# aje220/OptiMOBO

Measured on AMD Instinct MI355X. Metric: EHVI candidate evals/sec at n_train=512, 2-obj; 1/2/4/8-GPU scaling, higher is better.
Workload: dtype f64; 1 GPU; 2-obj EHVI (reference mode), ZDT1 surrogate, n_train=512, n_var=6, 2^20 Sobol candidates per GPU (BASELINE config 3); n_train=512, n_var=6, n_obj=2, candidates_per_gpu=1048576, global_batch=1048576, parallelism=dp1, train_box=x_1 in [0, 1], x_2..x_6 in [0, 0.3]

## Files before the change

### include/optimobo_hip.h

```cpp
#ifndef OPTIMOBO_HIP_H
#define OPTIMOBO_HIP_H

#include <stdint.h>

#ifdef __cplusplus
extern "C" {
#endif

#define OMB_ABI_VERSION 1
#define OMB_MAX_OBJ 8
#define OMB_MAX_DIM 256
#define OMB_MAX_TRAIN 1024
#define OMB_MAX_TRAIN_DENSE 16384
#define OMB_HVI_PATHS_CHUNK 262144
#define OMB_NONDOM_SETS 16
#define OMB_NONDOM_POINTS 16777216

enum {
  OMB_OK = 0,
  OMB_EINVAL = -1,
  OMB_EHIP = -2,
  OMB_ENOMEM = -3,
  OMB_ESTATE = -4,
  OMB_EUNSUP = -5,
// ... 35 lines not shown
  OMB_DEBUG_COV_TABLE = 2,
  OMB_DEBUG_FUSED_CHAIN = 3,
  OMB_DEBUG_ARGMAX_PASSES = 4,
  OMB_DEBUG_CHOL_MODE = 5,
  OMB_DEBUG_TIMING_STRIDE = 6,
  OMB_DEBUG_COV_FUSED = 8,
  OMB_DEBUG_SELECT_SEQ = 9,
  OMB_DEBUG_SYRK_GLDS = 10,
  OMB_DEBUG_BOXES_KD = 11,
  OMB_DEBUG_POSTERIOR_ALL_VAR = 12,
  OMB_DEBUG_POSTERIOR_MEAN_KERNEL = 13,
  OMB_DEBUG_PATHS_LIBCOS = 14,
  OMB_DEBUG_HVI_PATHS_CHUNK = 15,
  OMB_DEBUG_ARGMAX_PRUNE = 16,
  OMB_DEBUG_ARGMAX_SCREEN = 17,
  OMB_DEBUG_ARGMAX_STAGED = 18
};
int omb_debug_set(omb_ctx* ctx, int what, int64_t value);

int omb_set_gp(omb_ctx* ctx, int obj, int kernel, int n, int d, const double* X_dev,
               const double* lengthscale_host, double variance, const double* alpha_dev,
               const double* Linv_dev);

int omb_kernel_block(omb_ctx* ctx, int obj, const double* Xc_dev, int64_t N, double* K_dev);

int omb_posterior(omb_ctx* ctx, int n_obj, const double* Xc_dev, int64_t N, double* mu_dev,
                  double* var_dev);

int omb_posterior_screen(omb_ctx* ctx, const double* Xc_dev, int64_t N, int n_obj, double* mu_out_dev,
                          double* eps_out_dev);

// ... 24 lines not shown
                  int C, const int32_t* box_off_host, const uint16_t* boxes_dev, double* out_dev);
int omb_hvi_paths_grad(omb_ctx* ctx, int k, int S, int d, const double* y_dev, const double* dy_dev, int64_t ld,
                       int64_t N, const double* coords_dev, int C, const int32_t* box_off_host,
                       const uint16_t* boxes_dev, double* out_dev, double* grad_dev, double* t_dev,
                       double* tgrad_dev);
#define OMB_CON_VIOLATION 1u
int omb_hvi_paths_con(omb_ctx* ctx, int k, int S, int n_con, const double* y_dev, int64_t ld, int64_t N,
                      const double* coords_dev, int C, const int32_t* box_off_host, const uint16_t* boxes_dev,
                      double eta, unsigned flags, double* out_dev, double* u_dev);

int omb_nondominated(omb_ctx* ctx, int k, int S, const double* y_dev, int64_t ld, int64_t N, uint8_t* mask_dev,
                     int64_t ldm, int64_t* count_dev);
int omb_nondominated_stats(omb_ctx* ctx, int64_t* survivors_host, int* rounds_host);
int omb_argmax_prune_stats(omb_ctx* ctx, int64_t* stats_host);
int omb_argmax_stage_stats(omb_ctx* ctx, int64_t* stats_host);

int omb_hvpoi(omb_ctx* ctx, const double* mu_dev, const double* var_dev, int64_t ld, int64_t N,
              const double* cells_dev, int C, double* out_dev);

int omb_expdec(omb_ctx* ctx, int k, const double* mu_dev, const double* var_dev, int64_t ld, int64_t N,
               const double* cache_dev, int M, int scal_id, const double* params_host,
               const double* weights_host, const double* ideal_host, const double* max_host,
               double agg_min, double* out_dev);

int omb_ei(omb_ctx* ctx, const double* mu_dev, const double* var_dev, int64_t N, double best,
           double var_eps, double* out_dev);
int omb_ei_ext(omb_ctx* ctx, int kind, int k, const double* mu_dev, const double* var_dev, int64_t ld, int64_t N,
               double best, double var_eps, double pof_eps, double* out_dev);

int omb_feasibility(omb_ctx* ctx, int c, const double* mu_dev, const double* var_dev, int64_t ld, int64_t N,
// ... 97 lines not shown
```

### optimobo_amd/_lib.py

```python
import ctypes
import os

HERE = os.path.dirname(os.path.abspath(__file__))
LIB_PATH = os.environ.get("OMB_LIB_PATH") or os.path.join(HERE, "liboptimobo_hip.so")

OMB_OK, OMB_EINVAL, OMB_EHIP, OMB_ENOMEM, OMB_ESTATE, OMB_EUNSUP, OMB_ENOTPD = 0, -1, -2, -3, -4, -5, -6
ERROR_NAMES = {OMB_EINVAL: "OMB_EINVAL", OMB_EHIP: "OMB_EHIP", OMB_ENOMEM: "OMB_ENOMEM",
               OMB_ESTATE: "OMB_ESTATE", OMB_EUNSUP: "OMB_EUNSUP", OMB_ENOTPD: "OMB_ENOTPD"}
KERNEL_MATERN52, KERNEL_RBF = 0, 1
EHVI_REFERENCE, EHVI_TEXTBOOK, EHVI_SIGMA = 0, 1, 2
EI_PLAIN, EI_PARETO, EI_CONSTRAINED = 0, 1, 2
EA_EI, EA_PARETO_EI = 0, 1
DEBUG_SPIN_LIMIT = 1
DEBUG_COV_TABLE = 2
DEBUG_FUSED_CHAIN = 3
DEBUG_ARGMAX_PASSES = 4
DEBUG_CHOL_MODE = 5
DEBUG_TIMING_STRIDE = 6
DEBUG_COV_FUSED = 8
DEBUG_SELECT_SEQ = 9
DEBUG_SYRK_GLDS = 10
DEBUG_BOXES_KD = 11
DEBUG_POSTERIOR_ALL_VAR = 12
DEBUG_POSTERIOR_MEAN_KERNEL = 13
DEBUG_PATHS_LIBCOS = 14
DEBUG_HVI_PATHS_CHUNK = 15
DEBUG_ARGMAX_PRUNE = 16
DEBUG_ARGMAX_SCREEN = 17
DEBUG_ARGMAX_STAGED = 18
MAX_OBJ, MAX_DIM, MAX_TRAIN, MAX_TRAIN_DENSE = 8, 256, 1024, 16384
CON_VIOLATION = 1
HVI_PATHS_CHUNK = 1 << 18
NONDOM_SETS = 16
NONDOM_POINTS = 1 << 24

_p = ctypes.c_void_p
_d = ctypes.c_double
_i = ctypes.c_int
_i64 = ctypes.c_int64
_dp = ctypes.POINTER(ctypes.c_double)

SIGNATURES = {
    "omb_abi_version": (_i, []),
    "omb_create": (_i, [_i, ctypes.POINTER(_p)]),
# ... 9 lines not shown
    "omb_posterior_screen": (_i, [_p, _p, _i64, _i, _p, _p]),
    "omb_posterior_screen_list": (_i, [_p, _p, _i64, _p, _p, _i, _p, _p]),
    "omb_ehvi2d": (_i, [_p, _p, _p, _i64, _i64, _p, _i, _dp, _d, _d, _i, _p]),
    "omb_ehvi3d_mc": (_i, [_p, _p, _p, _i64, _i64, _p, _i, _dp, _d, _p, _p]),
    "omb_ehvi_mc": (_i, [_p, _i, _p, _p, _i64, _i64, _p, _i, _dp, _d, _p, _p]),
    "omb_ehvi_boxes": (_i, [_p, _i, _p, _p, _i64, _i64, _p, _i, _p, _i, _p]),
    "omb_ehvi_boxes_k": (_i, [_p, _i, _p, _p, _i64, _i64, _p, _i, _p, _i, _p]),
    "omb_hvi_boxes": (_i, [_p, _i, _p, _i64, _i64, _p, _i, _p, _i, _p]),
    "omb_hvi_paths": (_i, [_p, _i, _i, _p, _i64, _i64, _p, _i, _p, _p, _p]),
    "omb_hvi_paths_grad": (_i, [_p, _i, _i, _i, _p, _p, _i64, _i64, _p, _i, _p, _p, _p, _p, _p, _p]),
    "omb_hvi_paths_con": (_i, [_p, _i, _i, _i, _p, _i64, _i64, _p, _i, _p, _p, _d, ctypes.c_uint, _p, _p]),
    "omb_nondominated": (_i, [_p, _i, _i, _p, _i64, _i64, _p, _i64, _p]),
    "omb_nondominated_stats": (_i, [_p, ctypes.POINTER(_i64), ctypes.POINTER(_i)]),
    "omb_argmax_prune_stats": (_i, [_p, ctypes.POINTER(_i64)]),
    "omb_argmax_stage_stats": (_i, [_p, ctypes.POINTER(_i64)]),
    "omb_hvpoi": (_i, [_p, _p, _p, _i64, _i64, _p, _i, _p]),
    "omb_expdec": (_i, [_p, _i, _p, _p, _i64, _i64, _p, _i, _i, _dp, _dp, _dp, _dp, _d, _p]),
    "omb_ei": (_i, [_p, _p, _p, _i64, _d, _d, _p]),
    "omb_ei_ext": (_i, [_p, _i, _i, _p, _p, _i64, _i64, _d, _d, _d, _p]),
    "omb_feasibility": (_i, [_p, _i, _p, _p, _i64, _i64, _d, _p, _p]),
    "omb_log_ei": (_i, [_p, _i, _i, _p, _p, _i64, _i64, _d, _d, _d, _p]),
    "omb_log_ehvi_boxes": (_i, [_p, _i, _p, _p, _i64, _i64, _p, _i, _p, _i, _p]),
    "omb_log_feasibility": (_i, [_p, _i, _p, _p, _i64, _i64, _d, _p, _p]),
    "omb_mes": (_i, [_p, _i, _p, _p, _i64, _i64, _p, _i, _p]),
    "omb_argmax_dev": (_i, [_p, _p, _i64, _i64, _p]),
    "omb_argmax": (_i, [_p, _p, _i64, _i64, _dp, ctypes.POINTER(_i64)]),
    "omb_plan_ehvi2d": (_i, [_p, _p, _i, _dp, _d, _d, _i]),
    "omb_plan_ehvi3d_mc": (_i, [_p, _p, _i, _dp, _d]),
    "omb_plan_ehvi_mc": (_i, [_p, _i, _p, _i, _dp, _d]),
    "omb_plan_ehvi_boxes": (_i, [_p, _i, _p, _i, _p, _i]),
# ... 72 lines not shown
```

### optimobo_amd/csrc/omb_acquisition.hip

```cpp
#include <math.h>

#include "omb_internal.h"
#include "omb_math.h"

namespace omb {

constexpr int kAcqThreads = 256;

static unsigned acq_grid(int64_t N) {
  int64_t b = (N + kAcqThreads - 1) / kAcqThreads;
  if (b > 65536) b = 65536;
  return (unsigned)(b < 1 ? 1 : b);
}

int ehvi2d_lanes(int64_t N) { return N >= (1 << 19) ? 1 : (N >= (1 << 16) ? 2 : 4); }

template <int L>
__global__ __launch_bounds__(kAcqThreads) void ehvi2d_kernel(const double* __restrict__ mu,
                                                             const double* __restrict__ var, int64_t ld, int64_t N,
                                                             const double* __restrict__ pf, int P, double r0,
                                                             double r1, double s00, double s01, int mode,
                                                             double* __restrict__ out) {
  extern __shared__ double sm[];
  double* y1 = sm;
// ... 657 lines not shown
    off += (bytes + 15) / 16 * 16;
    return base ? base + o : nullptr;
  };
  ws->partials = reinterpret_cast<double*>(take(sizeof(double) * 2 * 2 * kArgmaxMaxBlocks));
  ws->tau = reinterpret_cast<double*>(take(sizeof(double) * 2));
  ws->counts = reinterpret_cast<int32_t*>(take(sizeof(int32_t) * 4));
  ws->seed_idx = reinterpret_cast<int32_t*>(take(sizeof(int32_t) * ((N + kPruneStride - 1) / kPruneStride)));
  ws->surv_idx = reinterpret_cast<int32_t*>(take(sizeof(int32_t) * N));
  ws->block_cnt = reinterpret_cast<int32_t*>(take(sizeof(int32_t) * ((N + kPruneBlock - 1) / kPruneBlock)));
  ws->keep = reinterpret_cast<uint8_t*>(take(N));
  ws->ubm = reinterpret_cast<double*>(take(sizeof(double) * N));
  ws->scr_mu = reinterpret_cast<double*>(take(sizeof(double) * 2 * N));
  ws->scr_eps = reinterpret_cast<double*>(take(sizeof(double) * 2 * N));
  ws->list_a = reinterpret_cast<int32_t*>(take(sizeof(int32_t) * N));
  ws->block_cnt_b = reinterpret_cast<int32_t*>(take(sizeof(int32_t) * ((N + kPruneBlock - 1) / kPruneBlock)));
  ws->stats_host = nullptr;
  return off;
}

int64_t prune_ws_bytes(int64_t N) {
  PruneWs ws;
  return prune_ws_layout(nullptr, N, &ws);
}

void prune_ws_carve(void* base, int64_t N, PruneWs* ws) { prune_ws_layout(static_cast<char*>(base), N, ws); }

__global__ __launch_bounds__(256) void prune_seed_kernel(int64_t ns, int32_t* __restrict__ seed_idx,
                                                         int32_t* __restrict__ counts) {
  for (int64_t j = (int64_t)blockIdx.x * blockDim.x + threadIdx.x; j < ns; j += (int64_t)gridDim.x * blockDim.x)
    seed_idx[j] = (int32_t)(j * kPruneStride);
// ... 346 lines not shown
      ubm[c] = v;
      const double score = -mc;
      if (score == score && argmax_better(score, c, bv, bi)) {
        bv = score;
        bi = c;
      }
    }
  }
  argmax_wave_block(bv, bi, red_v, red_i);
  if (threadIdx.x == 0) {
    seed_idx[blockIdx.x] = (int32_t)(bi < 0 ? first : bi);
    if (blockIdx.x == 0) counts[0] = (int32_t)gridDim.x;
  }
}

__global__ __launch_bounds__(kPruneBlock) void prune_bound_list_kernel(
    const double* __restrict__ mu0, const double* __restrict__ mu1, const double* __restrict__ eps0,
    const double* __restrict__ eps1, const int32_t* __restrict__ idx_a, const int32_t* __restrict__ count_a,
    int64_t cap, const double* __restrict__ pf, int P, double r0, double sA, double sB,
    const double* __restrict__ tau, uint8_t* __restrict__ keep, int32_t* __restrict__ block_cnt) {
#pragma clang fp contract(off)
  extern __shared__ double sm[];
  double* y1 = sm;
  double* y2 = sm + P + 1;
  __shared__ int wave_cnt[kPruneBlock / 64];
  const int64_t na = min((int64_t)*count_a, cap);
  if ((int64_t)blockIdx.x * kPruneBlock >= na) {
    if (threadIdx.x == 0) block_cnt[blockIdx.x] = 0;
    return;
  }
// ... 41 lines not shown
  for (int w = 0; w < wave; ++w) pos += wave_cnt[w];
  if (k) idx_b[pos] = idx_a[j];
}

hipError_t launch_prune_bound1_seed(hipStream_t stream, const double* mu1, const double* eps1, int64_t N,
                                    const double* pf, int P, double r0, double s00, double s01, double sf2,
                                    const double* alpha0, int n0, const PruneWs& ws) {
  const int64_t ng = (N + kPruneSeedGroup - 1) / kPruneSeedGroup;
  if (N < 1 || ng > (1 << 23) || !mu1 || !eps1 || !alpha0 || n0 < 0) return hipErrorInvalidValue;
  const size_t shm = sizeof(double) * (4 * P + 1);
  hipLaunchKernelGGL(prune_bound1_seed_kernel, dim3((unsigned)ng), dim3(kPruneBlock), shm, stream, mu1, eps1, N, pf, P,
                     r0, sf2 * s00, sf2 * s01, alpha0, n0, sf2, ws.ubm, ws.seed_idx, ws.counts);
  return hipGetLastError();
}

hipError_t launch_prune_threshold_a(hipStream_t stream, int64_t N, const PruneWs& ws) {
  PruneWs a = ws;
  a.surv_idx = ws.list_a;
  a.counts = ws.counts + 1;
  a.stats_host = ws.stats_host ? ws.stats_host + 1 : nullptr;
  return launch_prune_threshold(stream, N, a);
}

hipError_t launch_prune_bound_list(hipStream_t stream, const double* mu0, const double* mu1, const double* eps0,
                                   const double* eps1, int64_t cap, const double* pf, int P, double r0, double s00,
                                   double s01, double sf2, const PruneWs& ws) {
  const int64_t nb = (cap + kPruneBlock - 1) / kPruneBlock;
  if (cap < 1 || nb > (1 << 23) || !eps0 || !eps1) return hipErrorInvalidValue;
  const size_t shm = sizeof(double) * (2 * P + 1);
  hipLaunchKernelGGL(prune_bound_list_kernel, dim3((unsigned)nb), dim3(kPruneBlock), shm, stream, mu0, mu1, eps0, eps1,
                     ws.list_a, ws.counts + 2, cap, pf, P, r0, sf2 * s00, sf2 * s01, ws.tau, ws.keep, ws.block_cnt_b);
  hipError_t e = hipGetLastError();
  if (e != hipSuccess) return e;
  hipLaunchKernelGGL(prune_scan_kernel, dim3(1), dim3(1024), 0, stream, ws.block_cnt_b, (int)nb, ws.counts,
                     ws.stats_host);
  e = hipGetLastError();
// ... 8 lines not shown
```

### optimobo_amd/csrc/omb_api.hip

```cpp
#include <math.h>
#include <cmath>
#include <stdarg.h>
#include <stdio.h>
#include <string.h>

#include <new>
#include <string>
#include <vector>

#include "omb_internal.h"

using namespace omb;

struct ObjState {
  bool set = false;
  int n = 0, d = 0, DP = 0, R = 0, n_pad = 0, kind = 0;
  double variance = 0.0;
  double* buf = nullptr;
  size_t cap = 0;
  const double* Ld = nullptr;
  const double* Xraw = nullptr;
  double ls[OMB_MAX_DIM] = {};
  GPDev dev{};
  int path_S = 0, path_MT = 0;
// ... 67 lines not shown
  DevBuf ews;
  DevBuf fws;
  DevBuf dws;
  DevBuf gws;
  DevBuf aws;
  DevBuf hws;
  DevBuf pws;
  DevBuf nws;
  DevBuf nws2;
  DevBuf prws;
  int prune_taken = 0;
  int64_t prune_seed = 0;
  int64_t* prune_stats_host = nullptr;
  int64_t* prune_stats_dev = nullptr;
  int stage_taken = 0;
  int nd_rounds = 0;
  int64_t nd_survivors[kNdMaxRounds + 1] = {};
  int* fault_host = nullptr;
  int* fault_dev = nullptr;
  double* fit_host = nullptr;
  double* fit_dev = nullptr;
  int spin_limit = kDefaultSpinLimit;
  int cov_table = 0;
  int cov_fused = 1;
  int syrk_glds = 1;
  int fused_chain = 0;
  bool argmax_one_pass = false;
  int chol_mode = kCholPersistent;
  int chol_acq_rel = 0;
  int chol_single = 0;
  int select_seq = 0;
  int boxes_kd_wave = 0;
  int paths_libcos = 0;
  int hvi_paths_chunk = (int)kHviPathsChunk;
  int posterior_all_var = 0;
  int posterior_mean_kernel = kMeanKernelAfter;
  int argmax_prune = 1;
  int argmax_staged = 1;
  int argmax_screen = 1;
};

namespace {

int fail(omb_ctx* ctx, int code, const char* fmt, ...) {
  if (ctx) {
    char buf[512];
    va_list ap;
    va_start(ap, fmt);
    vsnprintf(buf, sizeof(buf), fmt, ap);
    va_end(ap);
    ctx->err = buf;
  }
  return code;
}
// ... 392 lines not shown
  const size_t head = paths ? (size_t)(k + pl.path_con) * pl.S * (size_t)Nc : 2 * (size_t)K * nd;
  const size_t doubles = head + nd + (nd + 1) / 2 + (sobol ? nd * args.d : 0);
  if ((rc = grow_dev(ctx, ctx->work, (doubles ? doubles : 1) * sizeof(double), "chain workspace"))) return rc;
  if (paths && N > 0) {
    const int64_t wsa = hvi_paths_ws_doubles(Nc, pl.S), wsb = hvi_paths_ws_doubles(N % Nc, pl.S);
    const int64_t wsd = wsa > wsb ? wsa : wsb;
    if (wsd && (rc = grow_dev(ctx, ctx->hws, sizeof(double) * (size_t)wsd, "HVI path workspace"))) return rc;
  }
  const bool two_phase = result_dev && !vals_out && !acq_raw && !all_var && !ctx->posterior_all_var && !paths &&
                         pl.kind == PLAN_EHVI2D && pl.prune_ok && pl.n_con == 0 && !pl.log && k == 2 &&
                         posterior_gather_fits(args, max_R) && N >= 1 && N <= kPruneMaxN &&
                         (ctx->argmax_prune >= 2 || (ctx->argmax_prune == 1 && N >= kPruneMinN));
  const bool seed_by_bound = ctx->argmax_prune != 2;
  const int64_t seed_step = seed_by_bound ? kPruneSeedGroup : kPruneStride;
  const bool staged = two_phase && seed_by_bound && ctx->argmax_screen != 0 && ctx->argmax_staged != 0;
  if (two_phase && (rc = grow_dev(ctx, ctx->prws, (size_t)prune_ws_bytes(N), "arg-max pruning workspace"))) return rc;
  if (result_dev) {
    ctx->prune_taken = two_phase ? 1 : 0;
    ctx->prune_seed = two_phase ? (N + seed_step - 1) / seed_step : 0;
    ctx->stage_taken = staged ? 1 : 0;
  }
  double* mu = ctx->work.as<double>();
  double* var = mu + (size_t)K * nd;
  double* vals = vals_out ? vals_out : mu + head;
  int32_t* raised = reinterpret_cast<int32_t*>(mu + head + nd);
  double* Xs = mu + head + nd + (nd + 1) / 2;
  double* acq = (pl.n_con && acq_raw) ? acq_raw : vals;

  hipEvent_t* ev = nullptr;
  if (ctx->timing && ctx->timing_calls++ % ctx->timing_stride == 0) {
    if (ctx->ev_used + 5 > ctx->ev.size() && ctx->ev.size() < 5 * 4096) {
      for (int i = 0; i < 5 * 64; ++i) {
        hipEvent_t e;
        OMB_HIP(ctx, hipEventCreate(&e));
        ctx->ev.push_back(e);
// ... 28 lines not shown
    PruneWs ws;
    prune_ws_carve(ctx->prws.p, N, &ws);
    ws.stats_host = ctx->prune_stats_dev;
    const int64_t ns = (N + seed_step - 1) / seed_step, nv = N - ns;
    const int nbs = prune_list_blocks(ns), nbv = nv > 0 ? prune_list_blocks(nv) : 0;
    double* mu_c = var;
    double* var_c = var + nd;
    const double sf2 = args.gp[0].variance;
    const bool screen = ctx->argmax_screen != 0;
    const double* bm = screen ? ws.scr_mu : mu;
    const double* be0 = screen ? ws.scr_eps : nullptr;
    const double* be1 = screen ? ws.scr_eps + nd : nullptr;
    if (e == hipSuccess && !screen) e = launch_posterior_means(ctx->stream, args, 3u, Xc, N, mu);
    if (e == hipSuccess && seed_by_bound && screen)
      e = launch_posterior_screen(ctx->stream, args, staged ? 2u : 3u, Xc, N, ws.scr_mu, ws.scr_eps);
    if (e == hipSuccess && staged)
      e = launch_prune_bound1_seed(ctx->stream, ws.scr_mu + nd, ws.scr_eps + nd, N, pl.geo, pl.P, pl.r[0], pl.s00,
                                   pl.s01, sf2, args.gp[0].alpha, args.gp[0].n, ws);
    if (e == hipSuccess && seed_by_bound && !staged)
      e = launch_prune_bound_seed(ctx->stream, bm, bm + nd, N, pl.geo, pl.P, pl.r[0], pl.s00, pl.s01, sf2, ws, be0,
                                  be1);
    if (e == hipSuccess && !seed_by_bound) e = launch_prune_seed(ctx->stream, N, ws);
    if (e == hipSuccess)
      e = launch_posterior_gather(ctx->stream, args, max_R, Xc, ws.seed_idx, ws.counts, ns, mu_c, var_c);
    if (e == hipSuccess && screen)
      e = launch_posterior_mean_gather(ctx->stream, args, 1, Xc, ws.seed_idx, ws.counts, ns, mu + nd);
    if (e == hipSuccess)
      e = launch_ehvi2d_argmax_list(ctx->stream, mu_c, var_c, mu + nd, ws.seed_idx, ws.counts, ns, pl.geo, pl.P,
                                    pl.r[0], pl.r[1], pl.s00, pl.s01, pl.mode, ws.partials);
    if (e == hipSuccess) e = launch_argmax_reduce(ctx->stream, ws.partials, nbs, 0, ws.tau);
    if (e == hipSuccess && seed_by_bound && !staged) e = launch_prune_threshold(ctx->stream, N, ws);
    if (staged && nv == 0) {
      if (e == hipSuccess) e = launch_prune_threshold_a(ctx->stream, N, ws);
      if (e == hipSuccess) e = launch_prune_threshold(ctx->stream, N, ws);
    } else if (staged) {
      if (e == hipSuccess) e = launch_prune_threshold_a(ctx->stream, N, ws);
      if (e == hipSuccess)
        e = launch_posterior_screen_gather(ctx->stream, args, 0, Xc, ws.list_a, ws.counts + 2, nv, ws.scr_mu,
                                           ws.scr_eps);
      if (e == hipSuccess)
        e = launch_prune_bound_list(ctx->stream, ws.scr_mu, ws.scr_mu + nd, ws.scr_eps, ws.scr_eps + nd, nv, pl.geo,
                                    pl.P, pl.r[0], pl.s00, pl.s01, sf2, ws);
    }
    if (e == hipSuccess && !seed_by_bound && screen)
      e = launch_posterior_screen(ctx->stream, args, 3u, Xc, N, ws.scr_mu, ws.scr_eps);
    if (e == hipSuccess && !seed_by_bound)
      e = launch_prune_bound(ctx->stream, bm, bm + nd, N, pl.geo, pl.P, pl.r[0], pl.s00, pl.s01, sf2, ws, be0, be1);
    if (e == hipSuccess && nv > 0)
      e = launch_posterior_gather(ctx->stream, args, max_R, Xc, ws.surv_idx, ws.counts + 1, nv, mu_c, var_c);
    if (e == hipSuccess && nv > 0 && screen)
      e = launch_posterior_mean_gather(ctx->stream, args, 1, Xc, ws.surv_idx, ws.counts + 1, nv, mu + nd);
// ... 43 lines not shown
  if (!ctx) return OMB_ENOMEM;
  ctx->device = device;
  if (hipSetDevice(device) != hipSuccess ||
      hipStreamCreateWithFlags(&ctx->own_stream, hipStreamNonBlocking) != hipSuccess ||
      hipMalloc(&ctx->partials, sizeof(double) * (2 * kArgmaxMaxBlocks + 2)) != hipSuccess ||
      hipMemset(ctx->partials, 0, sizeof(double) * (2 * kArgmaxMaxBlocks + 2)) != hipSuccess ||
      hipMalloc(&ctx->result_dev, sizeof(double) * 2) != hipSuccess ||
      hipHostMalloc(&ctx->result_host, sizeof(double) * 2, hipHostMallocDefault) != hipSuccess ||
      hipHostMalloc(&ctx->info_host, sizeof(int) * 4, hipHostMallocDefault) != hipSuccess ||
      hipMalloc(&ctx->sob, sobol_state_bytes(OMB_MAX_DIM, 32)) != hipSuccess ||
      hipHostMalloc(&ctx->fault_host, sizeof(int), hipHostMallocMapped | hipHostMallocCoherent) != hipSuccess ||
      hipHostGetDevicePointer(reinterpret_cast<void**>(&ctx->fault_dev), ctx->fault_host, 0) != hipSuccess ||
      hipHostMalloc(&ctx->fit_host, sizeof(double) * (OMB_MAX_DIM + 8), hipHostMallocMapped | hipHostMallocCoherent) !=
          hipSuccess ||
      hipHostGetDevicePointer(reinterpret_cast<void**>(&ctx->fit_dev), ctx->fit_host, 0) != hipSuccess ||
      hipHostMalloc(&ctx->prune_stats_host, sizeof(int64_t) * 2, hipHostMallocMapped | hipHostMallocCoherent) !=
          hipSuccess ||
      hipHostGetDevicePointer(reinterpret_cast<void**>(&ctx->prune_stats_dev), ctx->prune_stats_host, 0) !=
          hipSuccess) {
    omb_destroy(ctx);
    return OMB_ENOMEM;
  }
  *ctx->fault_host = 0;
  ctx->prune_stats_host[0] = ctx->prune_stats_host[1] = 0;
  ctx->stream = ctx->own_stream;
  *out = ctx;
  return OMB_OK;
}

int omb_destroy(omb_ctx* ctx) {
  if (!ctx) return OMB_OK;
  (void)hipSetDevice(ctx->device);
  if (ctx->stream) (void)hipStreamSynchronize(ctx->stream);
  for (auto& s : ctx->obj) {
    if (s.buf) (void)hipFree(s.buf);
    if (s.pbuf) (void)hipFree(s.pbuf);
  }
  if (ctx->partials) (void)hipFree(ctx->partials);
  if (ctx->result_dev) (void)hipFree(ctx->result_dev);
// ... 46 lines not shown
     "posterior mean kernel %lld (0 off, 1 after the posterior launch, 2 before it)"},
    {OMB_DEBUG_COV_TABLE, &omb_ctx::cov_table, 0, 1, nullptr},
    {OMB_DEBUG_COV_FUSED, &omb_ctx::cov_fused, 0, 1, nullptr},
    {OMB_DEBUG_SYRK_GLDS, &omb_ctx::syrk_glds, 0, 1, nullptr},
    {OMB_DEBUG_SELECT_SEQ, &omb_ctx::select_seq, 0, 1, nullptr},
    {OMB_DEBUG_BOXES_KD, &omb_ctx::boxes_kd_wave, 0, 1, nullptr},
    {OMB_DEBUG_PATHS_LIBCOS, &omb_ctx::paths_libcos, 0, 1, nullptr},
    {OMB_DEBUG_HVI_PATHS_CHUNK, &omb_ctx::hvi_paths_chunk, 0, 0x7fffffff,
     "sampled-front chain chunk %lld outside [0, 2^31) (0: one pass)"},
    {OMB_DEBUG_POSTERIOR_ALL_VAR, &omb_ctx::posterior_all_var, 0, 1, nullptr},
    {OMB_DEBUG_ARGMAX_PRUNE, &omb_ctx::argmax_prune, 0, 3,
     "arg-max pruning %lld (0 dense, 1 two-phase for large batches, 2 strided seed at any size, 3 seed by bound at "
     "any size)"},
    {OMB_DEBUG_ARGMAX_SCREEN, &omb_ctx::argmax_screen, 0, 1, nullptr},
    {OMB_DEBUG_ARGMAX_STAGED, &omb_ctx::argmax_staged, 0, 1, nullptr},
};

int omb_debug_set(omb_ctx* ctx, int what, int64_t value) {
  if (!ctx) return OMB_EINVAL;
  for (const DebugSwitch& s : kDebugSwitches) {
    if (s.code != what) continue;
    if (!s.msg) value = value != 0;
    else if (value < s.lo || value > s.hi) return fail(ctx, OMB_EINVAL, s.msg, (long long)value);
    ctx->*s.field = (int)value;
    return OMB_OK;
  }
  if (what == OMB_DEBUG_ARGMAX_PASSES) {
    if (value != 1 && value != 2) return fail(ctx, OMB_EINVAL, "arg-max passes %lld (1 or 2)", (long long)value);
    ctx->argmax_one_pass = value == 1;
    return OMB_OK;
// ... 414 lines not shown
  stats_host[0] = ctx->prune_taken;
  stats_host[1] = ctx->prune_seed;
  stats_host[2] = ctx->prune_taken ? __atomic_load_n(ctx->prune_stats_host, __ATOMIC_ACQUIRE) : 0;
  return OMB_OK;
}

int omb_argmax_stage_stats(omb_ctx* ctx, int64_t* stats_host) {
  if (!ctx) return OMB_EINVAL;
  if (!stats_host) return fail(ctx, OMB_EINVAL, "null output");
  stats_host[0] = ctx->stage_taken;
  stats_host[1] = ctx->stage_taken ? __atomic_load_n(ctx->prune_stats_host + 1, __ATOMIC_ACQUIRE) : 0;
  stats_host[2] = ctx->stage_taken ? __atomic_load_n(ctx->prune_stats_host, __ATOMIC_ACQUIRE) : 0;
  return OMB_OK;
}

int omb_hvpoi(omb_ctx* ctx, const double* mu_dev, const double* var_dev, int64_t ld, int64_t N,
              const double* cells_dev, int C, double* out_dev) {
  int rc = enter(ctx);
  if (rc) return rc;
  Plan pl;
  if ((rc = check_moments(E(ctx), mu_dev, var_dev, ld, N, 2, out_dev))) return rc;
  if (!cells_dev) return fail(ctx, OMB_EINVAL, "null cells");
  if ((rc = describe_hvpoi(ctx, C, &pl))) return rc;
  return run_acq(ctx, pl, cells_dev, nullptr, mu_dev, var_dev, ld, N, out_dev, nullptr, "hvpoi");
}

int omb_expdec(omb_ctx* ctx, int k, const double* mu_dev, const double* var_dev, int64_t ld, int64_t N,
               const double* cache_dev, int M, int scal_id, const double* params_host, const double* weights_host,
               const double* ideal_host, const double* max_host, double agg_min, double* out_dev) {
  int rc = enter(ctx);
// ... 996 lines not shown
```

### optimobo_amd/csrc/omb_internal.h

```cpp
#pragma once

#include <hip/hip_runtime.h>
#include <stdint.h>

#include "../../include/optimobo_hip.h"
#include "omb_host.h"
#include "omb_math.h"

namespace omb {

constexpr int kChunkRows = 64;
constexpr int kBlockThreads = 512;
constexpr int kKBlockRows = 256;

struct GPDev {
  const double* Xs;
  const double* xsq;
  const double* alpha;
  const double* Lp;
  const double* ls;
  double variance;
  int n;
  int R;
  int kind;
// ... 50 lines not shown
static_assert(kPruneSeedGroup % kPruneBlock == 0 && kPruneSeedGroup >= kPruneStride && kPruneSeedGroup <= 1024,
              "seed groups are whole workgroups of the threshold kernel and seed_idx holds ⌈N/kPruneStride⌉ entries");
struct PruneWs {
  int32_t* seed_idx;
  int32_t* surv_idx;
  int32_t* counts;
  int32_t* block_cnt;
  uint8_t* keep;
  double* ubm;
  double* scr_mu;
  double* scr_eps;
  double* partials;
  double* tau;
  int32_t* list_a;
  int32_t* block_cnt_b;
  int64_t* stats_host;
};
int64_t prune_ws_bytes(int64_t N);
void prune_ws_carve(void* base, int64_t N, PruneWs* ws);
hipError_t launch_prune_seed(hipStream_t stream, int64_t N, const PruneWs& ws);
int prune_list_blocks(int64_t cap);
hipError_t launch_ehvi2d_argmax_list(hipStream_t stream, const double* mu0_c, const double* var0_c, const double* mu1,
                                     const int32_t* idx, const int32_t* count, int64_t cap, const double* pf, int P,
                                     double r0, double r1, double s00, double s01, int mode, double* partials);
hipError_t launch_prune_bound(hipStream_t stream, const double* mu0, const double* mu1, int64_t N, const double* pf,
                              int P, double r0, double s00, double s01, double sf2, const PruneWs& ws,
                              const double* eps0 = nullptr, const double* eps1 = nullptr);
hipError_t launch_prune_bound_seed(hipStream_t stream, const double* mu0, const double* mu1, int64_t N,
                                   const double* pf, int P, double r0, double s00, double s01, double sf2,
                                   const PruneWs& ws, const double* eps0 = nullptr, const double* eps1 = nullptr);
hipError_t launch_prune_threshold(hipStream_t stream, int64_t N, const PruneWs& ws);
hipError_t launch_prune_bound1_seed(hipStream_t stream, const double* mu1, const double* eps1, int64_t N,
                                    const double* pf, int P, double r0, double s00, double s01, double sf2,
                                    const double* alpha0, int n0, const PruneWs& ws);
hipError_t launch_prune_threshold_a(hipStream_t stream, int64_t N, const PruneWs& ws);
hipError_t launch_prune_bound_list(hipStream_t stream, const double* mu0, const double* mu1, const double* eps0,
                                   const double* eps1, int64_t cap, const double* pf, int P, double r0, double s00,
                                   double s01, double sf2, const PruneWs& ws);

struct ArgmaxOut {
  double* partials;
  unsigned* ticket;
  double* result;
  int64_t offset;
};
int64_t ehvi2d_argmax_blocks(int64_t N);
hipError_t launch_ehvi2d_argmax(hipStream_t stream, const double* mu, const double* var, int64_t ld, int64_t N,
                                const double* pf, int P, double r0, double r1, double s00, double s01, int mode,
                                const ArgmaxOut& am);

// ... 241 lines not shown
```

### optimobo_amd/device.py

```python
import ctypes

import numpy as np
import torch

from . import _lib


_KERNEL_IDS = {"matern52": _lib.KERNEL_MATERN52, "rbf": _lib.KERNEL_RBF}
_EHVI_MODES = {"reference": _lib.EHVI_REFERENCE, "textbook": _lib.EHVI_TEXTBOOK, "sigma": _lib.EHVI_SIGMA}
_EI_KINDS = {"plain": _lib.EI_PLAIN, "pareto": _lib.EI_PARETO, "constrained": _lib.EI_CONSTRAINED}


def _ptr(t):
    return ctypes.c_void_p(t.data_ptr())


def _dev_f64(x, device):
    if isinstance(x, torch.Tensor):
        t = x.to(device=device, dtype=torch.float64)
    else:
        t = torch.as_tensor(np.ascontiguousarray(x, dtype=np.float64), device=device)
    return t.contiguous()


# ... 281 lines not shown
        surv = (ctypes.c_int64 * 5)()
        rounds = ctypes.c_int()
        self._check(self.lib.omb_nondominated_stats(self._h, surv, ctypes.byref(rounds)), "omb_nondominated_stats")
        return [int(v) for v in surv[:rounds.value]]

    def argmax_prune_stats(self):
        st = (ctypes.c_int64 * 3)()
        self._check(self.lib.omb_argmax_prune_stats(self._h, st), "omb_argmax_prune_stats")
        return bool(st[0]), int(st[1]), int(st[2])

    def argmax_stage_stats(self):
        st = (ctypes.c_int64 * 3)()
        self._check(self.lib.omb_argmax_stage_stats(self._h, st), "omb_argmax_stage_stats")
        return bool(st[0]), int(st[1]), int(st[2])

    def hvpoi(self, mu, var, cells, out=None):
        N = mu.shape[1]
        cells = _dev_f64(cells, self.device)
        out = self._out(out, N)
        self._stream()
        self._check(self.lib.omb_hvpoi(self._h, _ptr(mu), _ptr(var), mu.stride(0), N, _ptr(cells), cells.shape[0],
                                       _ptr(out)), "omb_hvpoi")
        return out

    def expdec(self, mu, var, cache, scal_id, params, weights, ideal, max_point, agg_min, out=None):
        k, N = mu.shape
        cache = _dev_f64(cache, self.device)
        out = self._out(out, N)
        self._stream()
        self._check(self.lib.omb_expdec(self._h, k, _ptr(mu), _ptr(var), mu.stride(0), N, _ptr(cache), cache.shape[0],
# ... 490 lines not shown
```

Before: 1.542 billion candidates/s.

## Replace per-candidate stage-1 bound with single solved mu1 cutoff for argmax pruning

In the staged argmax pruning path, the per-candidate EHVI upper bound on objective 1 is replaced by one scalar cutoff. A single-block kernel solves for that cutoff once against the current threshold using bracketing plus Newton-like iterations. Seeds are now chosen by lowest mu1 per group, and the threshold pass becomes a cheap comparison of mu1-eps1 against the cutoff. This removes the per-candidate loop over Pareto points in the first stage, at the cost of a serial solve kernel, a possibly looser filter that lets more candidates through, and careful rounding margins to keep pruning conservative.

New measurement: 1.690 billion candidates/s, median of 6. 9.6% higher.

```diff
diff --git a/include/optimobo_hip.h b/include/optimobo_hip.h
--- a/include/optimobo_hip.h
+++ b/include/optimobo_hip.h
@@ -73,7 +73,8 @@
   OMB_DEBUG_HVI_PATHS_CHUNK = 15,
   OMB_DEBUG_ARGMAX_PRUNE = 16,
   OMB_DEBUG_ARGMAX_SCREEN = 17,
-  OMB_DEBUG_ARGMAX_STAGED = 18
+  OMB_DEBUG_ARGMAX_STAGED = 18,
+  OMB_DEBUG_ARGMAX_CUT = 19
 };
 int omb_debug_set(omb_ctx* ctx, int what, int64_t value);
 
@@ -128,6 +129,7 @@
 int omb_nondominated_stats(omb_ctx* ctx, int64_t* survivors_host, int* rounds_host);
 int omb_argmax_prune_stats(omb_ctx* ctx, int64_t* stats_host);
 int omb_argmax_stage_stats(omb_ctx* ctx, int64_t* stats_host);
+int omb_argmax_cut_stats(omb_ctx* ctx, double* stats_host);
 
 int omb_hvpoi(omb_ctx* ctx, const double* mu_dev, const double* var_dev, int64_t ld, int64_t N,
               const double* cells_dev, int C, double* out_dev);
diff --git a/optimobo_amd/_lib.py b/optimobo_amd/_lib.py
--- a/optimobo_amd/_lib.py
+++ b/optimobo_amd/_lib.py
@@ -28,6 +28,7 @@
 DEBUG_ARGMAX_PRUNE = 16
 DEBUG_ARGMAX_SCREEN = 17
 DEBUG_ARGMAX_STAGED = 18
+DEBUG_ARGMAX_CUT = 19
 MAX_OBJ, MAX_DIM, MAX_TRAIN, MAX_TRAIN_DENSE = 8, 256, 1024, 16384
 CON_VIOLATION = 1
 HVI_PATHS_CHUNK = 1 << 18
@@ -67,6 +68,7 @@
     "omb_nondominated_stats": (_i, [_p, ctypes.POINTER(_i64), ctypes.POINTER(_i)]),
     "omb_argmax_prune_stats": (_i, [_p, ctypes.POINTER(_i64)]),
     "omb_argmax_stage_stats": (_i, [_p, ctypes.POINTER(_i64)]),
+    "omb_argmax_cut_stats": (_i, [_p, _dp]),
     "omb_hvpoi": (_i, [_p, _p, _p, _i64, _i64, _p, _i, _p]),
     "omb_expdec": (_i, [_p, _i, _p, _p, _i64, _i64, _p, _i, _i, _dp, _dp, _dp, _dp, _d, _p]),
     "omb_ei": (_i, [_p, _p, _p, _i64, _d, _d, _p]),
diff --git a/optimobo_amd/csrc/omb_acquisition.hip b/optimobo_amd/csrc/omb_acquisition.hip
--- a/optimobo_amd/csrc/omb_acquisition.hip
+++ b/optimobo_amd/csrc/omb_acquisition.hip
@@ -695,6 +695,7 @@
   ws->scr_eps = reinterpret_cast<double*>(take(sizeof(double) * 2 * N));
   ws->list_a = reinterpret_cast<int32_t*>(take(sizeof(int32_t) * N));
   ws->block_cnt_b = reinterpret_cast<int32_t*>(take(sizeof(int32_t) * ((N + kPruneBlock - 1) / kPruneBlock)));
+  ws->cut = reinterpret_cast<double*>(take(sizeof(double) * 4));
   ws->stats_host = nullptr;
   return off;
 }
@@ -1071,6 +1072,209 @@
   }
 }
 
+__global__ __launch_bounds__(kPruneBlock) void prune_seed1_kernel(const double* __restrict__ mu1, int64_t N,
+                                                                  int32_t* __restrict__ seed_idx,
+                                                                  int32_t* __restrict__ counts) {
+  __shared__ double red_v[kPruneBlock / 64];
+  __shared__ long long red_i[kPruneBlock / 64];
+  const int64_t first = (int64_t)blockIdx.x * kPruneSeedGroup;
+  double bv = -__builtin_inf();
+  long long bi = -1;
+  for (int j = 0; j < kPruneSeedGroup / kPruneBlock; ++j) {
+    const int64_t c = first + j * kPruneBlock + threadIdx.x;
+    if (c < N) {
+      const double score = -mu1[c];
+      if (score == score && argmax_better(score, c, bv, bi)) {
+        bv = score;
+        bi = c;
+      }
+    }
+  }
+  argmax_wave_block(bv, bi, red_v, red_i);
+  if (threadIdx.x == 0) {
+    seed_idx[blockIdx.x] = (int32_t)(bi < 0 ? first : bi);
+    if (blockIdx.x == 0) counts[0] = (int32_t)gridDim.x;
+  }
+}
+
+__device__ __forceinline__ double cut_ubm1(double m, const double* y2, const double* Ci, const double* Wi, int P,
+                                           int lane, double sB, double iB, double& D) {
+#pragma clang fp contract(off)
+  double ub = 0.0, scale = 0.0, d = 0.0;
+  for (int i = lane; i < P; i += 64) {
+    const double dy = y2[i] - m;
+    const double u = dy * iB;
+    const double cdf = ndtr_fast(u);
+    const double p2 = fmax(sB * npdf_fast(u) + dy * cdf, 0.0);
+    ub += Ci[i] * p2;
+    scale += p2 * Wi[i];
+    d += Ci[i] * cdf;
+  }
+  for (int o = 32; o > 0; o >>= 1) {
+    ub += __shfl_xor(ub, o);
+    scale += __shfl_xor(scale, o);
+    d += __shfl_xor(d, o);
+  }
+  D = d;
+  const double tiny = 64.0 * 0x1p-52 * scale + 1e-300;
+  return ub * (1.0 + 1e-9) + tiny;
+}
+
+constexpr int kCutBracketSteps = 64;
+constexpr int kCutSolveSteps = 64;
+constexpr int kCutWalkSteps = 3;
+__global__ __launch_bounds__(kPruneBlock) void prune_cut_kernel(const double* __restrict__ pf, int P, double r0,
+                                                                double sA, double sB,
+                                                                const double* __restrict__ alpha0, int n0,
+                                                                double var0, const double* __restrict__ tau,
+                                                                double* __restrict__ cut, int64_t* stats_host) {
+#pragma clang fp contract(off)
+  extern __shared__ double sm[];
+  double* y1 = sm;
+  double* y2 = sm + P + 1;
+  double* Ci = y2 + P;
+  double* Wi = Ci + P;
+  __shared__ double red_a[kPruneBlock / 64];
+  for (int i = threadIdx.x; i < P; i += blockDim.x) {
+    y1[i + 1] = pf[2 * i];
+    y2[i] = pf[2 * i + 1];
+  }
+  if (threadIdx.x == 0) y1[0] = r0;
+  double sa = 0.0;
+  for (int k = threadIdx.x; k < n0; k += blockDim.x) sa += fabs(alpha0[k]);
+  for (int o = 32; o > 0; o >>= 1) sa += __shfl_xor(sa, o);
+  if ((threadIdx.x & 63) == 0) red_a[threadIdx.x >> 6] = sa;
+  __syncthreads();
+  double M0 = 0.0;
+  for (int w = 0; w < kPruneBlock / 64; ++w) M0 += red_a[w];
+  M0 = var0 * M0 * (1.0 + 0x1p-20);
+  const double iA = 1.0 / sA, iB = 1.0 / sB;
+  for (int i = threadIdx.x; i < P; i += blockDim.x) {
+    const double a = y1[i], b = y1[i + 1];
+    const double dab = a - b, t = dab * iA;
+    Ci[i] = sA * npdf_fast(t) + dab * ndtr_fast(t);
+    Wi[i] = fabs(a) + fabs(b) + 2.0 * M0 + sA;
+  }
+  __syncthreads();
+  if (threadIdx.x >= 64) return;
+  const int lane = threadIdx.x;
+  const double inf = __builtin_inf();
+  const double t = tau[0];
+  bool fin = fabs(M0) < inf;
+  double ymax = -inf, ymin = inf;
+  for (int i = lane; i < P; i += 64) {
+    fin = fin && fabs(Ci[i]) < inf && fabs(Wi[i]) < inf;
+    ymax = fmax(ymax, y2[i]);
+    ymin = fmin(ymin, y2[i]);
+  }
+  for (int o = 32; o > 0; o >>= 1) {
+    ymax = fmax(ymax, __shfl_xor(ymax, o));
+    ymin = fmin(ymin, __shfl_xor(ymin, o));
+  }
+  fin = __all(fin) != 0 && fabs(ymax) < inf && fabs(ymin) < inf;
+  double hi = inf, uhi = __builtin_nan(""), lo = -inf;
+  if (fin && t > 0.0) {
+    double D;
+    double f = cut_ubm1(ymax, y2, Ci, Wi, P, lane, sB, iB, D);
+    double mN = ymax, fN = f, DN = D;
+    bool have_lo = false;
+    if (f < t) {
+      hi = ymax;
+      uhi = f;
+      double step = (ymax - ymin) + sB;
+      for (int k = 0; k < kCutBracketSteps && !have_lo; ++k) {
+        const double m = ymax - step;
+        step = 2.0 * step;
+        f = cut_ubm1(m, y2, Ci, Wi, P, lane, sB, iB, D);
+        if (f < t) {
+          hi = m;
+          uhi = f;
+          mN = m;
+          fN = f;
+          DN = D;
+        } else {
+          lo = m;
+          have_lo = true;
+        }
+      }
+    } else {
+      lo = ymax;
+      have_lo = true;
+      const double m = ymax + 40.0 * sB;
+      f = cut_ubm1(m, y2, Ci, Wi, P, lane, sB, iB, D);
+      if (f < t) {
+        hi = m;
+        uhi = f;
+      }
+    }
+    if (have_lo && hi < inf) {
+      const double tt = t * (1.0 - 5e-8), tw = t * (1.0 - 1e-7);
+      bool done = uhi >= tw;
+      for (int k = 0; k < kCutSolveSteps && !done; ++k) {
+        double m = mN + fN * log(fN / tt) / (DN * (1.0 + 1e-9));
+        if (!(m > lo && m < hi)) m = lo + 0.5 * (hi - lo);
+        if (!(m > lo && m < hi)) break;
+        f = cut_ubm1(m, y2, Ci, Wi, P, lane, sB, iB, D);
+        mN = m;
+        fN = f;
+        DN = D;
+        if (f < t) {
+          hi = m;
+          uhi = f;
+          done = f >= tw;
+        } else {
+          lo = m;
+        }
+      }
+      for (int k = 0; k < kCutWalkSteps; ++k) {
+        const double m = nextafter(hi, -inf);
+        if (!(m > lo)) break;
+        f = cut_ubm1(m, y2, Ci, Wi, P, lane, sB, iB, D);
+        if (!(f < t)) break;
+        hi = m;
+        uhi = f;
+      }
+    }
+  }
+  if (lane == 0) {
+    cut[0] = hi;
+    cut[1] = t;
+    cut[2] = uhi;
+    if (stats_host) {
+      long long* sh = reinterpret_cast<long long*>(stats_host);
+      __hip_atomic_store(sh, __builtin_bit_cast(long long, hi), __ATOMIC_RELAXED, __HIP_MEMORY_SCOPE_SYSTEM);
+      __hip_atomic_store(sh + 1, __builtin_bit_cast(long long, t), __ATOMIC_RELAXED, __HIP_MEMORY_SCOPE_SYSTEM);
+      __hip_atomic_store(sh + 2, __builtin_bit_cast(long long, uhi), __ATOMIC_RELAXED, __HIP_MEMORY_SCOPE_SYSTEM);
+    }
+  }
+}
+
+__global__ __launch_bounds__(kPruneBlock) void prune_threshold_cut_kernel(const double* __restrict__ mu1,
+                                                                          const double* __restrict__ eps1,
+                                                                          const int32_t* __restrict__ seed_idx,
+                                                                          const double* __restrict__ cut, int64_t N,
+                                                                          uint8_t* __restrict__ keep,
+                                                                          int32_t* __restrict__ block_cnt) {
+#pragma clang fp contract(off)
+  __shared__ int wave_cnt[kPruneBlock / 64];
+  const int64_t c = (int64_t)blockIdx.x * kPruneBlock + threadIdx.x;
+  const double ms = cut[0];
+  bool k = false;
+  if (c < N) {
+    const double m1 = mu1[c] - eps1[c];
+    k = c != (int64_t)seed_idx[c / kPruneSeedGroup] && !(ms < __builtin_inf() && m1 >= ms);
+    keep[c] = k ? 1 : 0;
+  }
+  const int nw = __popcll(__ballot(k));
+  if ((threadIdx.x & 63) == 0) wave_cnt[threadIdx.x >> 6] = nw;
+  __syncthreads();
+  if (threadIdx.x == 0) {
+    int s = 0;
+    for (int w = 0; w < kPruneBlock / 64; ++w) s += wave_cnt[w];
+    block_cnt[blockIdx.x] = s;
+  }
+}
+
 __global__ __launch_bounds__(kPruneBlock) void prune_bound_list_kernel(
     const double* __restrict__ mu0, const double* __restrict__ mu1, const double* __restrict__ eps0,
     const double* __restrict__ eps1, const int32_t* __restrict__ idx_a, const int32_t* __restrict__ count_a,
@@ -1142,12 +1346,36 @@
   return hipGetLastError();
 }
 
-hipError_t launch_prune_threshold_a(hipStream_t stream, int64_t N, const PruneWs& ws) {
+hipError_t launch_prune_seed1(hipStream_t stream, const double* mu1, int64_t N, const PruneWs& ws) {
+  const int64_t ng = (N + kPruneSeedGroup - 1) / kPruneSeedGroup;
+  if (N < 1 || ng > (1 << 23) || !mu1) return hipErrorInvalidValue;
+  hipLaunchKernelGGL(prune_seed1_kernel, dim3((unsigned)ng), dim3(kPruneBlock), 0, stream, mu1, N, ws.seed_idx,
+                     ws.counts);
+  return hipGetLastError();
+}
+
+hipError_t launch_prune_cut(hipStream_t stream, const double* pf, int P, double r0, double s00, double s01, double sf2,
+                            const double* alpha0, int n0, const PruneWs& ws) {
+  if (P < 0 || !alpha0 || n0 < 0) return hipErrorInvalidValue;
+  const size_t shm = sizeof(double) * (4 * P + 1);
+  hipLaunchKernelGGL(prune_cut_kernel, dim3(1), dim3(kPruneBlock), shm, stream, pf, P, r0, sf2 * s00, sf2 * s01, alpha0,
+                     n0, sf2, ws.tau, ws.cut, ws.stats_host ? ws.stats_host + 2 : nullptr);
+  return hipGetLastError();
+}
+
+hipError_t launch_prune_threshold_a(hipStream_t stream, int64_t N, const PruneWs& ws, const double* mu1,
+                                    const double* eps1) {
   PruneWs a = ws;
   a.surv_idx = ws.list_a;
   a.counts = ws.counts + 1;
   a.stats_host = ws.stats_host ? ws.stats_host + 1 : nullptr;
-  return launch_prune_threshold(stream, N, a);
+  if (!mu1) return launch_prune_threshold(stream, N, a);
+  const int64_t nb = (N + kPruneBlock - 1) / kPruneBlock;
+  if (N < 1 || nb > (1 << 23) || !eps1) return hipErrorInvalidValue;
+  hipLaunchKernelGGL(prune_threshold_cut_kernel, dim3((unsigned)nb), dim3(kPruneBlock), 0, stream, mu1, eps1,
+                     ws.seed_idx, ws.cut, N, a.keep, a.block_cnt);
+  const hipError_t e = hipGetLastError();
+  return e != hipSuccess ? e : launch_prune_compact(stream, N, a);
 }
 
 hipError_t launch_prune_bound_list(hipStream_t stream, const double* mu0, const double* mu1, const double* eps0,
diff --git a/optimobo_amd/csrc/omb_api.hip b/optimobo_amd/csrc/omb_api.hip
--- a/optimobo_amd/csrc/omb_api.hip
+++ b/optimobo_amd/csrc/omb_api.hip
@@ -105,6 +105,7 @@
   int64_t* prune_stats_host = nullptr;
   int64_t* prune_stats_dev = nullptr;
   int stage_taken = 0;
+  int cut_taken = 0;
   int nd_rounds = 0;
   int64_t nd_survivors[kNdMaxRounds + 1] = {};
   int* fault_host = nullptr;
@@ -129,6 +130,7 @@
   int argmax_prune = 1;
   int argmax_staged = 1;
   int argmax_screen = 1;
+  int argmax_cut = 1;
 };
 
 namespace {
@@ -551,11 +553,13 @@
   const bool seed_by_bound = ctx->argmax_prune != 2;
   const int64_t seed_step = seed_by_bound ? kPruneSeedGroup : kPruneStride;
   const bool staged = two_phase && seed_by_bound && ctx->argmax_screen != 0 && ctx->argmax_staged != 0;
+  const bool cut = staged && ctx->argmax_cut != 0;
   if (two_phase && (rc = grow_dev(ctx, ctx->prws, (size_t)prune_ws_bytes(N), "arg-max pruning workspace"))) return rc;
   if (result_dev) {
     ctx->prune_taken = two_phase ? 1 : 0;
     ctx->prune_seed = two_phase ? (N + seed_step - 1) / seed_step : 0;
     ctx->stage_taken = staged ? 1 : 0;
+    ctx->cut_taken = cut ? 1 : 0;
   }
   double* mu = ctx->work.as<double>();
   double* var = mu + (size_t)K * nd;
@@ -614,7 +618,8 @@
     if (e == hipSuccess && !screen) e = launch_posterior_means(ctx->stream, args, 3u, Xc, N, mu);
     if (e == hipSuccess && seed_by_bound && screen)
       e = launch_posterior_screen(ctx->stream, args, staged ? 2u : 3u, Xc, N, ws.scr_mu, ws.scr_eps);
-    if (e == hipSuccess && staged)
+    if (e == hipSuccess && cut) e = launch_prune_seed1(ctx->stream, ws.scr_mu + nd, N, ws);
+    if (e == hipSuccess && staged && !cut)
       e = launch_prune_bound1_seed(ctx->stream, ws.scr_mu + nd, ws.scr_eps + nd, N, pl.geo, pl.P, pl.r[0], pl.s00,
                                    pl.s01, sf2, args.gp[0].alpha, args.gp[0].n, ws);
     if (e == hipSuccess && seed_by_bound && !staged)
@@ -630,11 +635,15 @@
                                     pl.r[0], pl.r[1], pl.s00, pl.s01, pl.mode, ws.partials);
     if (e == hipSuccess) e = launch_argmax_reduce(ctx->stream, ws.partials, nbs, 0, ws.tau);
     if (e == hipSuccess && seed_by_bound && !staged) e = launch_prune_threshold(ctx->stream, N, ws);
+    if (e == hipSuccess && cut)
+      e = launch_prune_cut(ctx->stream, pl.geo, pl.P, pl.r[0], pl.s00, pl.s01, sf2, args.gp[0].alpha, args.gp[0].n, ws);
+    const double* cm = cut ? ws.scr_mu + nd : nullptr;
+    const double* ce = cut ? ws.scr_eps + nd : nullptr;
     if (staged && nv == 0) {
-      if (e == hipSuccess) e = launch_prune_threshold_a(ctx->stream, N, ws);
+      if (e == hipSuccess) e = launch_prune_threshold_a(ctx->stream, N, ws, cm, ce);
       if (e == hipSuccess) e = launch_prune_threshold(ctx->stream, N, ws);
     } else if (staged) {
-      if (e == hipSuccess) e = launch_prune_threshold_a(ctx->stream, N, ws);
+      if (e == hipSuccess) e = launch_prune_threshold_a(ctx->stream, N, ws, cm, ce);
       if (e == hipSuccess)
         e = launch_posterior_screen_gather(ctx->stream, args, 0, Xc, ws.list_a, ws.counts + 2, nv, ws.scr_mu,
                                            ws.scr_eps);
@@ -708,7 +717,7 @@
       hipHostMalloc(&ctx->fit_host, sizeof(double) * (OMB_MAX_DIM + 8), hipHostMallocMapped | hipHostMallocCoherent) !=
           hipSuccess ||
       hipHostGetDevicePointer(reinterpret_cast<void**>(&ctx->fit_dev), ctx->fit_host, 0) != hipSuccess ||
-      hipHostMalloc(&ctx->prune_stats_host, sizeof(int64_t) * 2, hipHostMallocMapped | hipHostMallocCoherent) !=
+      hipHostMalloc(&ctx->prune_stats_host, sizeof(int64_t) * 5, hipHostMallocMapped | hipHostMallocCoherent) !=
           hipSuccess ||
       hipHostGetDevicePointer(reinterpret_cast<void**>(&ctx->prune_stats_dev), ctx->prune_stats_host, 0) !=
           hipSuccess) {
@@ -716,7 +725,7 @@
     return OMB_ENOMEM;
   }
   *ctx->fault_host = 0;
-  ctx->prune_stats_host[0] = ctx->prune_stats_host[1] = 0;
+  for (int i = 0; i < 5; ++i) ctx->prune_stats_host[i] = 0;
   ctx->stream = ctx->own_stream;
   *out = ctx;
   return OMB_OK;
@@ -793,6 +802,7 @@
      "any size)"},
     {OMB_DEBUG_ARGMAX_SCREEN, &omb_ctx::argmax_screen, 0, 1, nullptr},
     {OMB_DEBUG_ARGMAX_STAGED, &omb_ctx::argmax_staged, 0, 1, nullptr},
+    {OMB_DEBUG_ARGMAX_CUT, &omb_ctx::argmax_cut, 0, 1, nullptr},
 };
 
 int omb_debug_set(omb_ctx* ctx, int what, int64_t value) {
@@ -1237,6 +1247,19 @@
   return OMB_OK;
 }
 
+int omb_argmax_cut_stats(omb_ctx* ctx, double* stats_host) {
+  if (!ctx) return OMB_EINVAL;
+  if (!stats_host) return fail(ctx, OMB_EINVAL, "null output");
+  stats_host[0] = ctx->cut_taken;
+  for (int i = 0; i < 3; ++i) {
+    const int64_t bits = __atomic_load_n(ctx->prune_stats_host + 2 + i, __ATOMIC_ACQUIRE);
+    double v;
+    memcpy(&v, &bits, sizeof(v));
+    stats_host[1 + i] = ctx->cut_taken ? v : 0.0;
+  }
+  return OMB_OK;
+}
+
 int omb_hvpoi(omb_ctx* ctx, const double* mu_dev, const double* var_dev, int64_t ld, int64_t N,
               const double* cells_dev, int C, double* out_dev) {
   int rc = enter(ctx);
diff --git a/optimobo_amd/csrc/omb_internal.h b/optimobo_amd/csrc/omb_internal.h
--- a/optimobo_amd/csrc/omb_internal.h
+++ b/optimobo_amd/csrc/omb_internal.h
@@ -88,6 +88,7 @@
   double* tau;
   int32_t* list_a;
   int32_t* block_cnt_b;
+  double* cut;
   int64_t* stats_host;
 };
 int64_t prune_ws_bytes(int64_t N);
@@ -107,7 +108,11 @@
 hipError_t launch_prune_bound1_seed(hipStream_t stream, const double* mu1, const double* eps1, int64_t N,
                                     const double* pf, int P, double r0, double s00, double s01, double sf2,
                                     const double* alpha0, int n0, const PruneWs& ws);
-hipError_t launch_prune_threshold_a(hipStream_t stream, int64_t N, const PruneWs& ws);
+hipError_t launch_prune_threshold_a(hipStream_t stream, int64_t N, const PruneWs& ws, const double* mu1 = nullptr,
+                                    const double* eps1 = nullptr);
+hipError_t launch_prune_seed1(hipStream_t stream, const double* mu1, int64_t N, const PruneWs& ws);
+hipError_t launch_prune_cut(hipStream_t stream, const double* pf, int P, double r0, double s00, double s01, double sf2,
+                            const double* alpha0, int n0, const PruneWs& ws);
 hipError_t launch_prune_bound_list(hipStream_t stream, const double* mu0, const double* mu1, const double* eps0,
                                    const double* eps1, int64_t cap, const double* pf, int P, double r0, double s00,
                                    double s01, double sf2, const PruneWs& ws);
diff --git a/optimobo_amd/device.py b/optimobo_amd/device.py
--- a/optimobo_amd/device.py
+++ b/optimobo_amd/device.py
@@ -319,6 +319,11 @@
         self._check(self.lib.omb_argmax_stage_stats(self._h, st), "omb_argmax_stage_stats")
         return bool(st[0]), int(st[1]), int(st[2])
 
+    def argmax_cut_stats(self):
+        st = (ctypes.c_double * 4)()
+        self._check(self.lib.omb_argmax_cut_stats(self._h, st), "omb_argmax_cut_stats")
+        return bool(st[0]), float(st[1]), float(st[2]), float(st[3])
+
     def hvpoi(self, mu, var, cells, out=None):
         N = mu.shape[1]
         cells = _dev_f64(cells, self.device)
```
